# bigmat18/cuda-mesh-voxelization

Hardware: AMD Instinct MI355X
Metric: Mvoxels/s (voxelize+JFA) at N=512, bunny 1.35M tris (higher is better)
Workload: dtype f32

## Files before the change

cuda_mesh_voxelization_amd/build.py:

```python
from __future__ import annotations

import os
import shutil
import subprocess

PKG = os.path.dirname(os.path.abspath(__file__))
ROOT = os.path.dirname(PKG)
CSRC = os.path.join(PKG, "csrc")
LIB = os.path.join(PKG, "libvphip.so")
CLI = os.path.join(PKG, "vpcli")

HIP_SOURCES = ["capi.hip", "vox.hip", "csg.hip", "jfa_seed.hip", "jfa_first_two.hip", "jfa_dense.hip", "extract.hip", "multi.hip", "cvox.hip", "fill.hip", "morph.hip", "components.hip", "surfnets.hip", "edt.hip", "meshdist.hip", "isonets.hip", "winding.hip", "thickness.hip", "octree.hip", "skeleton.hip", "geodesic.hip"]
DENSE_PARTS = 10
HOOK_SOURCES = ["vox.hip", "multi.hip", "cvox.hip", "meshdist.hip"]
HOOKS_LIB = os.path.join(PKG, "libvphip_hooks.so")
HIP_FLAGS = ["--offload-arch=gfx950", "-O3", "-std=c++17", "-ffp-contract=off", "-fPIC", "-shared",
             "-Wall", "-Wno-unused-function"]


def _hipcc() -> str:
    exe = shutil.which("hipcc") or "/opt/rocm/bin/hipcc"
    if not os.path.exists(exe):
        raise RuntimeError("hipcc not found: cannot build libvphip.so")
    return exe


def _newer(target: str, sources) -> bool:
    if not os.path.exists(target):
        return True
    t = os.path.getmtime(target)
    return any(os.path.getmtime(s) > t for s in sources)


def _jobs(n: int) -> int:
    env = os.environ.get("VP_BUILD_JOBS")
    if env:
        return max(1, min(int(env), n))
    return max(1, min(8, max(2, (os.cpu_count() or 4) - 1), n))


def build_lib(force: bool = False, verbose: bool = False, hooks: bool = False) -> str:
    srcs = [os.path.join(CSRC, s) for s in HIP_SOURCES]
    deps = srcs + [os.path.join(CSRC, "vp_internal.h"), os.path.join(CSRC, "jfa_common.h"), os.path.join(CSRC, "wg_scan.h"), os.path.join(CSRC, "skeleton_simple.h"), os.path.join(ROOT, "include", "vphip.h")]
    objdir = os.path.join(PKG, "build")
    flags = [f for f in HIP_FLAGS if f != "-shared"]

    def link(objs, out):
        cmd = [_hipcc(), "--offload-arch=gfx950", "-shared", "-fPIC"] + objs + ["-o", out]
        if verbose:
            print(" ".join(cmd))
        subprocess.check_call(cmd)

    objs = []
    for s_ in srcs:
        base = os.path.basename(s_)
        if base == "jfa_dense.hip":
            objs += [os.path.join(objdir, "jfa_dense.hip.part%d.o" % part) for part in range(1, DENSE_PARTS + 1)]
        else:
            objs.append(os.path.join(objdir, base + ".o"))
    if force or _newer(LIB, deps) or (hooks and (force or _newer(HOOKS_LIB, deps + [LIB])) and not all(os.path.exists(o) for o in objs)):
        from concurrent.futures import ThreadPoolExecutor
        os.makedirs(objdir, exist_ok=True)
        cmds = []
        for s_ in srcs:
            base = os.path.basename(s_)
# ... 45 lines not shown
```

cuda_mesh_voxelization_amd/capi.py:

```python
from __future__ import annotations

import ctypes
import os

PKG = os.path.dirname(os.path.abspath(__file__))
LIB_PATH = os.environ.get("VPHIP_LIB") or os.path.join(PKG, "libvphip.so")
HOOKS_LIB_PATH = os.path.join(PKG, "libvphip_hooks.so")

ALGO_NAIVE, ALGO_TILED = 1, 2
OP_VOID, OP_UNION, OP_INTERSECTION, OP_DIFFERENCE = 0, 1, 2, 3
MORPH_DILATE, MORPH_ERODE, MORPH_OPEN, MORPH_CLOSE = 0, 1, 2, 3
EDT_SEEDS_SET, EDT_SEEDS_UNSET, EDT_SEEDS_BORDER = 0, 1, 2
EDT_NONE = 0xFFFFFFFF
MESH_NONE = 0xFFFFFFFF
ISO_LINEAR, ISO_SIGNED_SQUARE = 0, 1
CONN_6, CONN_26 = 6, 26
SKEL_KERNEL, SKEL_CURVE = 0, 1
GEO_6, GEO_26, GEO_CHAMFER = 0, 1, 2
GEO_NONE = 0xFFFFFFFF
COMP_KEEP_LARGEST, COMP_MIN_VOXELS = 0, 1
EXTRACT_SET, EXTRACT_EXPOSED, EXTRACT_FACES = 0, 1, 2
MULTI_HALO, MULTI_GHOST, MULTI_HYBRID, MULTI_TRANSPOSE = 0, 1, 2, 3

KERNELS = ["vox_setup", "vox_scan", "vox_scatter", "vox_tile", "vox_naive", "vox_fill",
# ... 388 lines not shown

    def release(self):
        check(lib().vp_ctx_release(self._h))

    def jfa_init(self, frame: Frame, d_words: int, d_below, d_above, d_ids: int):
        check(lib().vp_jfa_init(self._h, ctypes.byref(frame), _vp(d_words), _vp(d_below or None),
                                _vp(d_above or None), _vp(d_ids)))

    def jfa_pass(self, frame: Frame, k: int, d_in: int, d_minus, d_plus, d_out: int, algo: int = ALGO_TILED):
        check(lib().vp_jfa_pass(self._h, ctypes.byref(frame), k, _vp(d_in), _vp(d_minus or None),
                                _vp(d_plus or None), _vp(d_out), algo))

    def jfa_finalize(self, frame: Frame, d_words: int, d_ids: int, fill: float, d_sdf: int):
        check(lib().vp_jfa_finalize(self._h, ctypes.byref(frame), _vp(d_words), _vp(d_ids), fill, _vp(d_sdf)))

    def jfa_last_pass(self, frame: Frame, d_in: int, d_minus, d_plus, d_scratch: int, d_words: int, fill: float, d_sdf: int,
                      algo: int = ALGO_TILED):
        check(lib().vp_jfa_last_pass(self._h, ctypes.byref(frame), _vp(d_in), _vp(d_minus or None), _vp(d_plus or None),
                                     _vp(d_scratch), _vp(d_words), fill, _vp(d_sdf), algo))

    def jfa_can_start_from_mask(self, frame: Frame, algo: int = ALGO_TILED) -> bool:
        return bool(lib().vp_jfa_can_start_from_mask(ctypes.byref(frame), algo))

    def jfa_can_fuse_first_two(self, frame: Frame, algo: int = ALGO_TILED) -> bool:
        return bool(lib().vp_jfa_can_fuse_first_two(ctypes.byref(frame), algo))

    def jfa_window_bytes(self, frame: Frame, planes: int) -> int:
        return int(lib().vp_jfa_window_bytes(ctypes.byref(frame), planes))

    def jfa_window_span(self, frame: Frame, planes: int, p0: int, p1: int):
        off, nb = (_sz * 2)(), (_sz * 2)()
        check(lib().vp_jfa_window_span(ctypes.byref(frame), planes, p0, p1, off, nb))
        return [(int(off[i]), int(nb[i])) for i in range(2) if nb[i]]

    def jfa_window_clear(self, frame: Frame, win: Window):
        check(lib().vp_jfa_window_clear(self._h, ctypes.byref(frame), ctypes.byref(win)))

    def jfa_window_init(self, frame: Frame, d_words: int, d_below, d_above, win: Window):
        check(lib().vp_jfa_window_init(self._h, ctypes.byref(frame), _vp(d_words), _vp(d_below or None), _vp(d_above or None), ctypes.byref(win)))

    def jfa_window_first_pass(self, frame: Frame, d_border_grid: int, win: Window):
        check(lib().vp_jfa_window_first_pass(self._h, ctypes.byref(frame), _vp(d_border_grid), ctypes.byref(win)))

    def jfa_window_first_two(self, frame: Frame, d_border_grid: int, win: Window):
        check(lib().vp_jfa_window_first_two(self._h, ctypes.byref(frame), _vp(d_border_grid), ctypes.byref(win)))

    def jfa_window_pass(self, frame: Frame, k: int, win_in: Window, win_out: Window, stride=None):
        check(lib().vp_jfa_window_pass(self._h, ctypes.byref(frame), k, ctypes.byref(win_in), ctypes.byref(win_out), k if stride is None else stride))

    def jfa_window_last_pass(self, frame: Frame, win_in: Window, win_scratch: Window, d_words_region: int, fill: float, d_sdf_region: int, stride: int = 1):
        check(lib().vp_jfa_window_last_pass(self._h, ctypes.byref(frame), ctypes.byref(win_in), ctypes.byref(win_scratch), stride,
                                            _vp(d_words_region), fill, _vp(d_sdf_region)))

    @staticmethod
    def jfa_cyclic_passes(frame: Frame, ranks: int) -> int:
        return int(lib().vp_jfa_cyclic_passes(ctypes.byref(frame), ranks))

    def jfa_window_first_two_cyclic(self, frame: Frame, d_border_grid: int, win: Window, ranks: int, rank: int):
        check(lib().vp_jfa_window_first_two_cyclic(self._h, ctypes.byref(frame), _vp(d_border_grid), ctypes.byref(win), ranks, rank))

    def jfa_window_pass_cyclic(self, frame: Frame, k: int, win_in: Window, win_out: Window, ranks: int, rank: int):
        check(lib().vp_jfa_window_pass_cyclic(self._h, ctypes.byref(frame), k, ctypes.byref(win_in), ctypes.byref(win_out), ranks, rank))

    def jfa_window_interleave(self, frame: Frame, win_in: Window, win_out: Window, ranks: int, count: int):
        check(lib().vp_jfa_window_interleave(self._h, ctypes.byref(frame), ctypes.byref(win_in), ctypes.byref(win_out), ranks, count))

    def surface(self, frame: Frame, d_words: int, d_below, d_above, d_border: int):
        check(lib().vp_surface(self._h, ctypes.byref(frame), _vp(d_words), _vp(d_below or None),
                               _vp(d_above or None), _vp(d_border)))

    def extract_count(self, frame: Frame, d_words: int, mode: int) -> int:
        n = ctypes.c_uint64()
        check(lib().vp_extract_count(self._h, ctypes.byref(frame), _vp(d_words), mode, ctypes.byref(n)))
        return int(n.value)

    def extract(self, frame: Frame, d_words: int, mode: int, d_sdf, d_records: int, d_values, capacity: int):
        check(lib().vp_extract(self._h, ctypes.byref(frame), _vp(d_words), mode, _vp(d_sdf or None), _vp(d_records),
                               _vp(d_values or None), capacity))

    def surfnets_count(self, frame: Frame, d_words: int, algo: int = ALGO_TILED):
        nv, nq = ctypes.c_uint64(), ctypes.c_uint64()
        check(lib().vp_surfnets_count(self._h, ctypes.byref(frame), _vp(d_words), algo, ctypes.byref(nv), ctypes.byref(nq)))
        return int(nv.value), int(nq.value)

    def surfnets(self, frame: Frame, d_words: int, algo: int, iterations: int, d_cells: int, d_xyz: int, d_quads: int,
                 vertex_capacity: int, quad_capacity: int):
        check(lib().vp_surfnets(self._h, ctypes.byref(frame), _vp(d_words), algo, iterations, _vp(d_cells or None), _vp(d_xyz or None),
                                _vp(d_quads or None), vertex_capacity, quad_capacity))

    def isonets(self, frame: Frame, d_field: int, transform: int = ISO_SIGNED_SQUARE, iso: float = 0.0, iterations: int = 0,
                normals: bool = False, algo: int = ALGO_TILED):
        nv, nq = ctypes.c_uint64(), ctypes.c_uint64()
        check(lib().vp_isonets(self._h, ctypes.byref(frame), _vp(d_field or None), transform, iso, iterations, 1 if normals else 0, algo,
                               ctypes.byref(nv), ctypes.byref(nq)))
        return int(nv.value), int(nq.value)

    def isonets_result(self):
        c, x, m, q = _vp(), _vp(), _vp(), _vp()
        nv, nq = ctypes.c_uint64(), ctypes.c_uint64()
        check(lib().vp_isonets_result(self._h, ctypes.byref(c), ctypes.byref(x), ctypes.byref(m), ctypes.byref(q), ctypes.byref(nv),
                                      ctypes.byref(nq)))
        return c.value or 0, x.value or 0, m.value or 0, q.value or 0, int(nv.value), int(nq.value)

    def winding(self, frame: Frame, d_xyz: int, nverts: int, d_tri: int, ntris: int, beta: float = 2.0, level: float = 0.5,
                algo: int = ALGO_TILED, count: bool = False):
        c = ctypes.c_uint64()
# ... 285 lines not shown
```

cuda_mesh_voxelization_amd/csrc/capi.hip:

```cpp
#include "vp_internal.h"

#include <algorithm>
#include <cmath>
#include <cstdarg>
#include <cstdio>
#include <cstring>
#include <initializer_list>

namespace vp {

static thread_local char g_err[512] = "";

int set_error(int code, const char* fmt, ...)
{
    va_list ap;
    va_start(ap, fmt);
    vsnprintf(g_err, sizeof(g_err), fmt, ap);
    va_end(ap);
    return code;
}

int hip_fail(hipError_t e, const char* what, const char* file, int line)
{
    snprintf(g_err, sizeof(g_err), "[%s:%d] HIP Assert: %s (%s)", file, line, hipGetErrorString(e), what);
// ... 664 lines not shown
        VP_TRY(reserve(ctx, ctx->jfa_work, vp_jfa_workspace_bytes(f)));
        if (ctx->jfa_work.ptr != before) ctx->jfa_started.valid = false;
        d_work = ctx->jfa_work.ptr;
        work_bytes = ctx->jfa_work.bytes;
    } else if (work_bytes < vp_jfa_workspace_bytes(f)) {
        return set_error(VP_ERR_INVALID, "%s: workspace too small", who);
    }
    return 0;
}

static bool jfa_tile_sequence(const Frame& fr, int algo) { return jfa_can_fuse_first_two(fr, algo) && fr.n / 4 >= 1; }

int vp_jfa_start(vp_ctx* ctx, const vp_frame* f, const uint32_t* d_words, void* d_work, size_t work_bytes, int algo)
{
    const bool explicitWork = d_work != nullptr;
    VP_TRY(jfa_check(ctx, f, d_words, d_work, work_bytes, algo, "vp_jfa_start"));
    const Frame fr = make_frame(f);
    const size_t volBytes = vp_grid_voxels(f) * vp_jfa_id_bytes(f);
    char* a = (char*)d_work;
    const bool mask = jfa_tile_sequence(fr, algo);
    ctx->jfa_started.valid = false;
    if (explicitWork) grid_written(ctx, d_work, vp_jfa_workspace_bytes(f));
    if (mask) VP_TRY(launch_jfa_init(ctx, fr, d_words, nullptr, nullptr, nullptr, (uint32_t*)(a + 2 * volBytes)));
    else      VP_TRY(launch_jfa_init(ctx, fr, d_words, nullptr, nullptr, a, nullptr));
    ctx->jfa_started = {true, mask, f->n, algo, d_work, work_bytes, d_words};
    return 0;
}

int vp_jfa_run(vp_ctx* ctx, const vp_frame* f, const uint32_t* d_words, float fill_unset, float* d_sdf,
               void* d_work, size_t work_bytes, int algo)
{
    if (!d_sdf) return set_error(VP_ERR_INVALID, "vp_jfa_run: null argument");
    VP_TRY(check_aligned("vp_jfa_run", {d_sdf}));
    const bool explicitWork = d_work != nullptr;
    VP_TRY(jfa_check(ctx, f, d_words, d_work, work_bytes, algo, "vp_jfa_run"));
    VP_TRY(check_fill(fill_unset, "vp_jfa_run"));
    const Frame fr = make_frame(f);
    const size_t volBytes = vp_grid_voxels(f) * vp_jfa_id_bytes(f);
    char* a = (char*)d_work;
    char* b = a + volBytes;
    uint32_t k = f->n / 2;
    const bool wantMask = jfa_tile_sequence(fr, algo);
    const vp_ctx::JfaStarted st = ctx->jfa_started;
    ctx->jfa_started.valid = false;
    if (!st.valid || st.n != f->n || st.algo != algo || st.work != d_work || st.words != d_words || st.mask != wantMask)
        return set_error(VP_ERR_INVALID, "vp_jfa_run: call vp_jfa_start with the same grid, frame, algo and workspace first");
    if (explicitWork) grid_written(ctx, d_work, vp_jfa_workspace_bytes(f));
    grid_written(ctx, d_sdf, vp_grid_voxels(f) * 4);
    if (wantMask) {
        IdWin wa, wb;
        wa.base = a; wb.base = b; wa.planes = wb.planes = f->n; wa.at = wb.at = 0;
        VP_TRY(launch_win_first_two(ctx, fr, (const uint32_t*)(b + volBytes), wa));
        for (k /= 4; k >= 1; k /= 2) {
            if (k == 1) return launch_win_pass(ctx, fr, 1, wa, wb, 1, d_words, fill_unset, d_sdf);
            VP_TRY(launch_win_pass(ctx, fr, k, wa, wb, k, nullptr, 0.0f, nullptr));
            std::swap(wa, wb);
        }
        return set_error(VP_ERR_INVALID, "vp_jfa_run: internal: no last pass");
    }
    for (; k >= 1; k /= 2) {
        if (k == 1 && jfa_pass_can_fuse_final(fr, k, algo))
            return launch_jfa_pass_ex(ctx, fr, k, a, nullptr, nullptr, b, algo, d_words, fill_unset, d_sdf);
        VP_TRY(launch_jfa_pass(ctx, fr, k, a, nullptr, nullptr, b, algo));
        char* t = a; a = b; b = t;
    }
    return launch_jfa_final(ctx, fr, d_words, a, fill_unset, d_sdf);
}

int vp_jfa(vp_ctx* ctx, const vp_frame* f, const uint32_t* d_words, float fill_unset, float* d_sdf,
           void* d_work, size_t work_bytes, int algo)
{
    if (!d_sdf) return set_error(VP_ERR_INVALID, "vp_jfa: null argument");
    VP_TRY(check_aligned("vp_jfa", {d_sdf}));
    VP_TRY(check_fill(fill_unset, "vp_jfa"));
    VP_TRY(vp_jfa_start(ctx, f, d_words, d_work, work_bytes, algo));
    return vp_jfa_run(ctx, f, d_words, fill_unset, d_sdf, d_work, work_bytes, algo);
}

size_t vp_jfa_state_bytes(const vp_frame* f, int algo)
{
    if (!f || check_frame(f, "vp_jfa_state_bytes", false) != 0) return 0;
    return (algo == VP_ALGO_TILED && win_compact(f->n)) ? 5 : vp_jfa_id_bytes(f);
}

int vp_jfa_last_shapes(const vp_ctx* ctx, vp_jfa_shape* out, int cap)
{
    if (!ctx) return 0;
    for (int i = 0; out && i < ctx->dense_shape_count && i < cap; ++i) out[i] = ctx->dense_shapes[i];
    return ctx->dense_shape_count;
}

int vp_jfa_can_start_from_mask(const vp_frame* f, int algo)
{
    return (f && check_frame(f, "vp_jfa_can_start_from_mask", false) == 0 && jfa_can_start_from_mask(make_frame(f), algo)) ? 1 : 0;
}

int vp_jfa_can_fuse_first_two(const vp_frame* f, int algo)
{
    return (f && check_frame(f, "vp_jfa_can_fuse_first_two", false) == 0 && jfa_can_fuse_first_two(make_frame(f), algo)) ? 1 : 0;
}

int vp_jfa_last_pass(vp_ctx* ctx, const vp_frame* f, const void* d_in, const void* d_minus, const void* d_plus,
                     void* d_scratch, const uint32_t* d_words, float fill_unset, float* d_sdf, int algo)
{
    if (ctx) ctx->dense_shape_count = 0;
    if (!ctx || !d_in || !d_scratch || !d_words || !d_sdf || d_in == d_scratch)
        return set_error(VP_ERR_INVALID, "vp_jfa_last_pass: bad buffers");
// ... 157 lines not shown
        return set_error(VP_ERR_INVALID, "%s: %llu planes at index %u do not fit a window of %u planes", who, (unsigned long long)planes, out->at, out->planes);
    if (overlaps(in->d_ids, win_bytes(f->n, in->planes), out->d_ids, win_bytes(f->n, out->planes))) return set_error(VP_ERR_INVALID, "%s: the two windows overlap", who);
    IdWin wi, wo;
    wi.base = (char*)in->d_ids; wi.planes = in->planes; wi.at = 0;
    wo.base = (char*)out->d_ids; wo.planes = out->planes; wo.at = out->at;
    window_written(ctx, out);
    return launch_win_interleave(ctx, f->n, wi, wo, ranks, count);
}

static void pass_reach(const vp_frame* f, uint32_t k, uint32_t stride, uint32_t& below, uint32_t& above)
{
    if (stride == k) {
        below = std::min(k, f->z0);
        above = std::min(k, f->n - f->z1);
    } else {
        below = f->z1 > k ? stride : 0;
        above = f->z0 + k < f->n ? stride : 0;
    }
}

static int window_pass(vp_ctx* ctx, const vp_frame* f, uint32_t k, const vp_window* in, const vp_window* out, uint32_t stride,
                       const uint32_t* d_words, float fill, float* d_sdf, const char* who)
{
    if (ctx) ctx->dense_shape_count = 0;
    if (!in || !out || !in->d_ids || !out->d_ids || in->d_ids == out->d_ids) return set_error(VP_ERR_INVALID, "%s: bad windows", who);
    if (in->planes != out->planes || in->at != out->at) return set_error(VP_ERR_INVALID, "%s: the two windows must have the same planes / at", who);
    if (f && f->n && overlaps(in->d_ids, win_bytes(f->n, in->planes), out->d_ids, win_bytes(f->n, out->planes)))
        return set_error(VP_ERR_INVALID, "%s: the two windows overlap", who);
    if (!f || k == 0 || k >= f->n) return set_error(VP_ERR_INVALID, "%s: step %u out of range", who, k);
    if (stride == 0 || (stride != k && (k < f->z1 - f->z0 || stride < f->z1 - f->z0)))
        return set_error(VP_ERR_INVALID, "%s: stride %u: either the step itself or, for a step of at least the slab height, the distance of the slabs in the window", who, stride);
    uint32_t below = 0, above = 0;
    pass_reach(f, k, stride, below, above);
    IdWin wi, wo;
    VP_TRY(window_check(ctx, f, in, who, below, above, wi));
    VP_TRY(window_check(ctx, f, out, who, 0, 0, wo));
    window_written(ctx, out);
    if (d_sdf) grid_written(ctx, d_sdf, vp_grid_voxels(f) * 4);
    return launch_win_pass(ctx, make_frame(f), k, wi, wo, stride, d_words, fill, d_sdf);
}

int vp_jfa_window_pass(vp_ctx* ctx, const vp_frame* f, uint32_t k, const vp_window* in, const vp_window* out, uint32_t stride)
{
    return window_pass(ctx, f, k, in, out, stride, nullptr, 0.0f, nullptr, "vp_jfa_window_pass");
}

int vp_jfa_window_last_pass(vp_ctx* ctx, const vp_frame* f, const vp_window* in, const vp_window* scratch, uint32_t stride,
                            const uint32_t* d_words_region, float fill_unset, float* d_sdf_region)
{
    if (!d_words_region || !d_sdf_region) return set_error(VP_ERR_INVALID, "vp_jfa_window_last_pass: null argument");
    VP_TRY(check_aligned("vp_jfa_window_last_pass", {d_words_region, d_sdf_region}));
    VP_TRY(check_fill(fill_unset, "vp_jfa_window_last_pass"));
    return window_pass(ctx, f, 1, in, scratch, stride, d_words_region, fill_unset, d_sdf_region, "vp_jfa_window_last_pass");
}

int vp_extract_count(vp_ctx* ctx, const vp_frame* f, const uint32_t* d_words, int mode, uint64_t* h_count)
{
    if (!ctx || !d_words) return set_error(VP_ERR_INVALID, "vp_extract_count: null argument");
    VP_TRY(bind_device(ctx));
    VP_TRY(check_frame(f, "vp_extract_count", true));
    if (mode < VP_EXTRACT_SET || mode > VP_EXTRACT_FACES) return set_error(VP_ERR_INVALID, "vp_extract_count: mode %d", mode);
    return launch_extract_count(ctx, make_frame(f), d_words, mode, h_count);
}

int vp_extract(vp_ctx* ctx, const vp_frame* f, const uint32_t* d_words, int mode, const float* d_sdf,
               uint64_t* d_records, float* d_values, size_t capacity)
{
    if (!ctx || !d_words || (!d_records && capacity)) return set_error(VP_ERR_INVALID, "vp_extract: null argument");
    if ((d_values != nullptr) != (d_sdf != nullptr)) return set_error(VP_ERR_INVALID, "vp_extract: d_sdf and d_values go together");
    VP_TRY(bind_device(ctx));
    VP_TRY(check_frame(f, "vp_extract", true));
    if (mode < VP_EXTRACT_SET || mode > VP_EXTRACT_FACES) return set_error(VP_ERR_INVALID, "vp_extract: mode %d", mode);
    const size_t cnt = (size_t)std::min<uint64_t>(capacity, ctx->ext_total);
    if (cnt) {
        grid_written(ctx, d_records, cnt * 8);
        grid_written(ctx, d_values, cnt * 4);
    }
    return launch_extract_write(ctx, make_frame(f), d_words, mode, d_sdf, d_records, d_values, capacity);
}

static int check_surfnets(const vp_frame* f, const char* who)
{
    VP_TRY(check_frame(f, who, false));
    VP_TRY(check_whole(f, who));
    if (f->n > 1024) return set_error(VP_ERR_UNSUPPORTED, "%s: n=%u is not served (32 <= n <= 1024: cell indices are 32-bit)", who, f->n);
    return 0;
}

int vp_surfnets_count(vp_ctx* ctx, const vp_frame* f, const uint32_t* d_words, int algo, uint64_t* h_vertices, uint64_t* h_quads)
{
    const char* who = "vp_surfnets_count";
    if (!ctx || !d_words || !h_vertices || !h_quads) return set_error(VP_ERR_INVALID, "%s: null argument", who);
    VP_TRY(bind_device(ctx));
    VP_TRY(check_surfnets(f, who));
    VP_TRY(check_algo(who, algo));
    VP_TRY(check_aligned(who, {d_words}));
    return launch_surfnets_count(ctx, f->n, d_words, algo, h_vertices, h_quads);
}

int vp_surfnets(vp_ctx* ctx, const vp_frame* f, const uint32_t* d_words, int algo, uint32_t iterations, uint64_t* d_cells, float* d_xyz,
                uint32_t* d_quads, size_t vertex_capacity, size_t quad_capacity)
{
    const char* who = "vp_surfnets";
    if (!ctx || !d_words) return set_error(VP_ERR_INVALID, "%s: null argument", who);
    VP_TRY(bind_device(ctx));
    VP_TRY(check_surfnets(f, who));
// ... 623 lines not shown
```

cuda_mesh_voxelization_amd/csrc/jfa_common.h:

```cpp
#pragma once
#include "vp_internal.h"
#include <algorithm>
#include <cstdlib>
#include <type_traits>

#pragma clang fp contract(off)

namespace vp {
namespace {

__device__ __forceinline__ uint32_t scr(uint32_t i) { return i ^ ((i >> 5) & 31u); }

__device__ __forceinline__ void udivmod(uint32_t a, uint32_t b, uint32_t& q, uint32_t& r)
{
    if ((b & (b - 1u)) == 0u) { q = a >> (uint32_t)__builtin_ctz(b); r = a & (b - 1u); }
    else { q = a / b; r = a % b; }
}

struct FastDiv {
    uint32_t d, m, s1, s2;
    __device__ __forceinline__ void divmod(uint32_t a, uint32_t& q, uint32_t& r) const
    {
        const uint32_t t = __umulhi(m, a);
        q = (t + ((a - t) >> s1)) >> s2;
// ... 53 lines not shown
    static constexpr int kTabZ = 3072;
    static constexpr uint32_t kMask = 0x1FFCu;
    static constexpr uint32_t kNoneWord = 0xFFFFF800u;
    static constexpr uint32_t kNoneBit = 4u;
    static constexpr uint32_t kNoneByte = 4u;
    __device__ static __forceinline__ T none() { return make_uint2(kNoneWord, kNoneByte); }
    __device__ static __forceinline__ bool is_none(T a) { return (a.y & kNoneBit) != 0u; }
    __device__ static __forceinline__ T pack(uint32_t x, uint32_t y, uint32_t z)
    {
        const uint32_t sz = scr(z);
        return make_uint2(x | (scr(y) << 11) | ((sz & 1023u) << 22), (sz >> 10) << 1);
    }
    __device__ static __forceinline__ T from64(uint2 a)
    {
        if (a.x == 0xFFFFFFFFu) return none();
        const uint32_t sz = (a.x >> 2) & 2047u, sy = (a.y >> 2) & 2047u;
        return make_uint2((a.x >> 13) | (sy << 11) | ((sz & 1023u) << 22), (sz >> 10) << 1);
    }
    __device__ static __forceinline__ uint32_t xoff(T a) { return (a.x & 0x7FFu) << 2; }
    __device__ static __forceinline__ uint32_t zoff(T a) { return ((a.x >> 20) & 0xFFCu) | (a.y << 11); }
    __device__ static __forceinline__ uint32_t yoff(T a) { return (a.x >> 9) & kMask; }
    __device__ static __forceinline__ uint32_t zt2(T a) { return a.y & 2u; }
};

__device__ __forceinline__ float axis_pos(float o, uint32_t i, float vs) { return o + ((float)(int)i * vs); }

template <class ID>
__device__ __forceinline__ float seed_distance(const Frame& f, typename ID::T id, float px, float py, float pz)
{
    const float sx = axis_pos(f.ox, ID::xoff(id) >> 2, f.vs);
    const float sy = axis_pos(f.oy, scr(ID::yoff(id) >> 2), f.vs);
    const float sz = axis_pos(f.oz, scr(ID::zoff(id) >> 2), f.vs);
    return ((sx - px) * (sx - px)) + ((sy - py) * (sy - py)) + ((sz - pz) * (sz - pz));
}

__device__ __forceinline__ __amdgpu_buffer_rsrc_t row_resource(const void* row, uint32_t bytes)
{
    return __builtin_amdgcn_make_buffer_rsrc(const_cast<void*>(row), 0, (int)bytes, 0x00020000);
}
__device__ __forceinline__ void row_load(uint32_t& o, __amdgpu_buffer_rsrc_t r, uint32_t byte_off)
{
    o = __builtin_amdgcn_raw_buffer_load_b32(r, (int)byte_off, 0, 0);
}
__device__ __forceinline__ void row_load(uint2& o, __amdgpu_buffer_rsrc_t r, uint32_t byte_off)
{
    const auto v = __builtin_amdgcn_raw_buffer_load_b64(r, (int)byte_off, 0, 0);
    o = make_uint2(v[0], v[1]);
}
__device__ __forceinline__ uint32_t row_load_u8(__amdgpu_buffer_rsrc_t r, uint32_t byte_off)
{
    return (uint32_t)__builtin_amdgcn_raw_buffer_load_b8(r, (int)byte_off, 0, 0);
}
__device__ __forceinline__ float lds_f32(const char* p) { return *reinterpret_cast<const float*>(p); }
template <int AUX = 0>
__device__ __forceinline__ void row_store(uint32_t v, __amdgpu_buffer_rsrc_t r, uint32_t byte_off)
{
    __builtin_amdgcn_raw_buffer_store_b32(v, r, (int)byte_off, 0, AUX);
}
template <int AUX = 0>
__device__ __forceinline__ void row_store(float v, __amdgpu_buffer_rsrc_t r, uint32_t byte_off)
{
    __builtin_amdgcn_raw_buffer_store_b32(__float_as_uint(v), r, (int)byte_off, 0, AUX);
}
template <int AUX = 0>
__device__ __forceinline__ void row_store(uint2 v, __amdgpu_buffer_rsrc_t r, uint32_t byte_off)
{
    typedef uint32_t u32x2 __attribute__((ext_vector_type(2)));
    const u32x2 t = {v.x, v.y};
    __builtin_amdgcn_raw_buffer_store_b64(t, r, (int)byte_off, 0, AUX);
}
template <int AUX = 0>
__device__ __forceinline__ void row_store_u8(uint32_t v, __amdgpu_buffer_rsrc_t r, uint32_t byte_off)
{
    __builtin_amdgcn_raw_buffer_store_b8((unsigned char)v, r, (int)byte_off, 0, AUX);
}
__device__ __forceinline__ const char* opaque_uniform(const char* p)
{
    uint64_t v = reinterpret_cast<uint64_t>(p);
    asm volatile("" : "+s"(v));
    return reinterpret_cast<const char*>(v);
}
__device__ __forceinline__ size_t opaque_uniform(size_t v)
{
    asm volatile("" : "+s"(v));
    return v;
}
__device__ __forceinline__ void pin(float& a) { asm volatile("" : "+v"(a)); }
__device__ __forceinline__ void pin(uint32_t& a) { asm volatile("" : "+v"(a)); }
__device__ __forceinline__ void pin(uint2& a) { asm volatile("" : "+v"(a.x), "+v"(a.y)); }

typedef uint32_t u32x2 __attribute__((ext_vector_type(2)));

__device__ __forceinline__ double min_f64(double a, double b)
{
    double r;
    asm("v_min_f64 %0, %1, %2" : "=v"(r) : "v"(a), "v"(b));
    return r;
}
__device__ __forceinline__ float min3_f32(float a, float b, float c)
{
    float r;
    asm("v_min3_f32 %0, %1, %2, %3" : "=v"(r) : "v"(a), "v"(b), "v"(c));
    return r;
}

__device__ __forceinline__ float min_f32(float a, float b)
// ... 21 lines not shown
```

cuda_mesh_voxelization_amd/csrc/jfa_dense.hip:

```cpp
#include "jfa_common.h"

namespace vp {
namespace {

template <class ID> constexpr bool final_mask_global() { return ID::kTab > 512; }
constexpr int kStoreAux = 2;
template <int PM>
__device__ __forceinline__ float from_partner(float v)
{
    constexpr int ctrl = PM == 1 ? 0xB1 : PM == 2 ? 0x4E : PM == 4 ? 0x141 : 0x128;
    return __builtin_bit_cast(float, __builtin_amdgcn_update_dpp(0, __builtin_bit_cast(int, v), ctrl, 0xf, 0xf, true));
}
template <class ID, int RY, int NT, bool FINAL>
constexpr int dense_waves()
{
    return std::is_same<ID, IdC>::value ? 4 : RY > 4 ? 4 : (FINAL && !final_mask_global<ID>()) ? (ID::kTab == 512 ? 5 : 4) : (ID::kTab == 512 || NT == 512) ? 6 : 4;
}
template <class ID, int RY, int CH, int NT, bool FINAL, int PM, int CLOSED = 0, bool FULL = false, bool CYC = false>
__global__ void __launch_bounds__(NT, (dense_waves<ID, RY, NT, FINAL>()))
jfa_pass_dense(Frame f, uint32_t kArg, uint32_t ka, const char* __restrict__ in, const char* __restrict__ inB, char* __restrict__ out, char* __restrict__ outB,
               const char* __restrict__ none_row, const uint32_t* __restrict__ words, float fill, float* __restrict__ sdf,
               uint32_t tilesY, uint32_t tiles, uint32_t splitTiles, uint32_t cyc)
{
    static_assert(!CYC || !FINAL, "the last pass (k = 1) is never a multiple of the rank count");
    using T = typename ID::T;
    constexpr bool CPT = std::is_same<ID, IdC>::value;
    constexpr uint32_t IDB = 4u;
    constexpr int TAB = ID::kTab;
    constexpr int PXT = CPT ? TAB : TAB + 1;
    constexpr int TABZ = CPT ? IdC::kTabZ : TAB;
    constexpr int HY = (CLOSED & 1) ? 0 : 1;
    constexpr bool CZ = (CLOSED & 2) != 0;
    constexpr int NR = RY + 2 * HY;
    static_assert(!CLOSED || !FINAL, "closed tiles: id passes");
    constexpr int NC = PM ? 2 : 3;
    constexpr int NI = NR * NC;
    constexpr int CHT = CPT ? 1 : CH;
    using B = typename std::conditional<FINAL, float, double>::type;
    __shared__ float PX[PXT];
    __shared__ float TY[RY][TAB];
    __shared__ float TZ[CHT][TABZ];
    __shared__ uint32_t RB[CPT ? (CH + 2) * NR : 1];
    constexpr bool GM = final_mask_global<ID>();
    __shared__ uint32_t WM[(FINAL && !GM) ? RY * CH * (TAB / 32) : 1];

    const int N = (int)f.n;
    const uint32_t k = FINAL ? 1u : kArg;
    const int K = (int)k;
    const int zsh = CYC ? (int)(cyc & 31u) : 0, zoff = CYC ? (int)(cyc >> 8) : 0;
    const int KZ = CYC ? K >> zsh : K, NZ = CYC ? N >> zsh : N;
    auto zglobal = [&](int l) { return CYC ? zoff + (l << zsh) : l; };
    const int nzl = (int)(f.z1 - f.z0);
    const uint32_t tid = threadIdx.x;
    const int nresY = min(K, N);
    const bool rev = ((31 - __builtin_clz(k)) & 1) != 0;
    uint32_t lin = blockIdx.x;
    const uint32_t total = tiles;
    uint32_t xpart = 0, xparts = 1;
    if (lin >= total - splitTiles) {
// ... 568 lines not shown
```

cuda_mesh_voxelization_amd/csrc/vp_internal.h:

```cpp
#pragma once

#include <hip/hip_runtime.h>
#include <cstddef>
#include <cstdint>
#include <vector>

#include "../../include/vphip.h"

namespace vp {

constexpr uint32_t kNone9 = 0xFF9FF200u;
constexpr uint32_t kNone10 = 0xFFDFFC00u;
constexpr int kTile = 8;
constexpr int kRecDwords = 20;

struct Frame {
    uint32_t n;
    uint32_t w;
    uint32_t z0, z1;
    float vs, ox, oy, oz;
};

inline Frame make_frame(const vp_frame* f)
{
// ... 147 lines not shown
int launch_morph(vp_ctx* ctx, uint32_t n, const uint32_t* d_words, uint32_t* d_out, int op, uint32_t radius, int algo);
int launch_edt(vp_ctx* ctx, const Frame& f, const uint32_t* d_words, int seeds, uint32_t* d_dist, int algo);
int launch_edt_sdf(vp_ctx* ctx, const Frame& f, const uint32_t* d_words, float fill, float* d_sdf, int algo);
int launch_edt_morph(vp_ctx* ctx, const Frame& f, const uint32_t* d_words, uint32_t* d_out, int op, uint32_t radius, int algo);
int launch_edt_thresh(vp_ctx* ctx, uint32_t n, const uint32_t* d_dist, uint32_t* d_out, uint32_t r2, int greater);
int launch_thickness(vp_ctx* ctx, const Frame& f, const uint32_t* d_words, uint32_t rmax, uint32_t thin2, int algo, uint64_t* h_thin_count);
int launch_octree(vp_ctx* ctx, const Frame& f, const uint32_t* d_words, int algo, uint64_t* h_nodes);
int launch_octree_expand(vp_ctx* ctx, const Frame& f, const uint32_t* d_nodes, uint64_t nodes, uint32_t* d_words, int algo);
int octree_validate(const uint32_t* h_nodes, uint64_t nodes, uint32_t n);
int launch_skeleton(vp_ctx* ctx, const Frame& f, const uint32_t* d_words, const uint32_t* d_anchor, int mode, uint32_t max_iters, int algo,
                    uint64_t* h_stats);
int launch_skeleton_table(vp_ctx* ctx, int algo, uint32_t* d_table);
void skeleton_table_cpu(int algo, uint32_t* h_table);
int launch_geodesic(vp_ctx* ctx, const Frame& f, const uint32_t* d_mask, const uint32_t* d_seeds, int metric, int algo, uint64_t* h_stats);
int launch_mesh_distance(vp_ctx* ctx, const Frame& f, const float* d_xyz, size_t nverts, const uint32_t* d_tri, size_t ntris,
                         const uint32_t* d_sign, uint32_t band, float* d_dist, uint32_t* d_nearest, int algo);
int launch_winding(vp_ctx* ctx, const Frame& f, const float* d_xyz, size_t nverts, const uint32_t* d_tri, size_t ntris, float beta, float level,
                   int algo, uint64_t* h_inside_count);
int launch_components_label(vp_ctx* ctx, uint32_t n, const uint32_t* d_words, uint32_t* d_labels, int conn, int algo, uint32_t* h_count);
int launch_components_sizes(vp_ctx* ctx, uint32_t n, const uint32_t* d_labels, uint32_t count, uint32_t* d_sizes);
int launch_components_filter(vp_ctx* ctx, uint32_t n, const uint32_t* d_words, uint32_t* d_out, int conn, int mode, uint32_t param, int algo,
                             uint32_t* h_count, uint64_t* h_kept);
int launch_surfnets_count(vp_ctx* ctx, uint32_t n, const uint32_t* d_words, int algo, uint64_t* h_vertices, uint64_t* h_quads);
struct IsoField { const float* d_field; int transform; float iso; float* d_normals; };
int launch_surfnets_write(vp_ctx* ctx, uint32_t n, const uint32_t* d_words, int algo, uint32_t iterations, uint64_t* d_cells, float* d_xyz,
                          uint32_t* d_quads, const IsoField* iso = nullptr);
int launch_isonets(vp_ctx* ctx, uint32_t n, const float* d_field, int transform, float iso, uint32_t iterations, bool want_normals, int algo);
int launch_iso_place(vp_ctx* ctx, uint32_t n, int algo, const IsoField& iso, const uint64_t* d_cells, const uint32_t* index, float* d_xyz,
                     size_t nverts);
int launch_csg(vp_ctx* ctx, uint32_t* d_a, const uint32_t* d_b, size_t nwords, int op);
int launch_stream_copy(vp_ctx* ctx, void* d_dst, const void* d_src, size_t bytes);
size_t jfa_id_bytes(const Frame& f);
int launch_jfa_init(vp_ctx* ctx, const Frame& f, const uint32_t* d_words, const uint32_t* below,
                    const uint32_t* above, void* d_ids, uint32_t* d_border_words);
int launch_jfa_pass(vp_ctx* ctx, const Frame& f, uint32_t k, const void* d_in, const void* d_minus,
                    const void* d_plus, void* d_out, int algo);
bool jfa_pass_can_fuse_final(const Frame& f, uint32_t k, int algo);
int launch_jfa_pass_ex(vp_ctx* ctx, const Frame& f, uint32_t k, const void* d_in, const void* d_minus,
                       const void* d_plus, void* d_out, int algo, const uint32_t* d_words, float fill, float* d_sdf);
int launch_jfa_final(vp_ctx* ctx, const Frame& f, const uint32_t* d_words, const void* d_ids,
                     float fill, float* d_sdf);
bool jfa_can_start_from_mask(const Frame& f, int algo);
bool jfa_can_fuse_first_two(const Frame& f, int algo);
int launch_win_init(vp_ctx* ctx, const Frame& f, const uint32_t* d_words, const uint32_t* below, const uint32_t* above, const IdWin& out);
int launch_win_first_pass(vp_ctx* ctx, const Frame& f, const uint32_t* d_border, const IdWin& out);
int launch_win_clear(vp_ctx* ctx, uint32_t n, const IdWin& w);
int launch_win_pass(vp_ctx* ctx, const Frame& f, uint32_t k, const IdWin& in, const IdWin& out, uint32_t stride,
                    const uint32_t* d_words, float fill, float* d_sdf);
#define VP_DENSE_DECL(NAME) int NAME(vp_ctx* ctx, const Frame& f, uint32_t k, const IdWin& in, const IdWin& out, uint32_t stride, const uint32_t* d_words, float fill, float* d_sdf)
VP_DENSE_DECL(launch_dense_id9_pass);  VP_DENSE_DECL(launch_dense_id9_last);
VP_DENSE_DECL(launch_dense_id10_pass); VP_DENSE_DECL(launch_dense_id10_last);
VP_DENSE_DECL(launch_dense_idc_pass);  VP_DENSE_DECL(launch_dense_idc_last);
#undef VP_DENSE_DECL
int launch_win_first_two(vp_ctx* ctx, const Frame& f, const uint32_t* d_border, const IdWin& out, uint32_t ranks = 1, uint32_t rank = 0);
uint32_t jfa_cyclic_passes(uint32_t n, uint32_t ranks);
int launch_win_pass_cyclic(vp_ctx* ctx, const Frame& f, uint32_t k, const IdWin& in, const IdWin& out, uint32_t ranks, uint32_t rank);
#define VP_CYCLIC_DECL(NAME) int NAME(vp_ctx* ctx, const Frame& f, uint32_t k, const IdWin& in, const IdWin& out, uint32_t ranks, uint32_t rank)
VP_CYCLIC_DECL(launch_cyclic_id9_pass); VP_CYCLIC_DECL(launch_cyclic_id10_pass); VP_CYCLIC_DECL(launch_cyclic_idc_pass);
#undef VP_CYCLIC_DECL
int launch_win_interleave(vp_ctx* ctx, uint32_t n, const IdWin& in, const IdWin& out, uint32_t ranks, uint32_t count);
int launch_extract_count(vp_ctx* ctx, const Frame& f, const uint32_t* d_words, int mode, uint64_t* h_count);
int launch_extract_write(vp_ctx* ctx, const Frame& f, const uint32_t* d_words, int mode, const float* d_sdf,
                         uint64_t* d_records, float* d_values, size_t capacity);

}
```

Measured before the change: 51160.

## Add dedicated lane-vectorized kernel for the final JFA pass on whole grids

Adds a specialized kernel for the final k=1 JFA pass on whole power-of-two grids (256/512/1024). Each thread owns four consecutive x voxels loaded with 16-byte buffer loads and writes signed distances with 16-byte stores. The kernel rolls through z planes, reusing neighbour rows across planes, and precomputes squared y/z distance tables in LDS. It replaces the generic dense final pass whenever the id window and sdf are 16-byte aligned, trading higher register pressure and more code for fewer memory transactions and less redundant arithmetic.

```diff
diff --git a/cuda_mesh_voxelization_amd/build.py b/cuda_mesh_voxelization_amd/build.py
--- a/cuda_mesh_voxelization_amd/build.py
+++ b/cuda_mesh_voxelization_amd/build.py
@@ -10,7 +10,7 @@
 LIB = os.path.join(PKG, "libvphip.so")
 CLI = os.path.join(PKG, "vpcli")
 
-HIP_SOURCES = ["capi.hip", "vox.hip", "csg.hip", "jfa_seed.hip", "jfa_first_two.hip", "jfa_dense.hip", "extract.hip", "multi.hip", "cvox.hip", "fill.hip", "morph.hip", "components.hip", "surfnets.hip", "edt.hip", "meshdist.hip", "isonets.hip", "winding.hip", "thickness.hip", "octree.hip", "skeleton.hip", "geodesic.hip"]
+HIP_SOURCES = ["capi.hip", "vox.hip", "csg.hip", "jfa_seed.hip", "jfa_first_two.hip", "jfa_dense.hip", "jfa_last.hip", "extract.hip", "multi.hip", "cvox.hip", "fill.hip", "morph.hip", "components.hip", "surfnets.hip", "edt.hip", "meshdist.hip", "isonets.hip", "winding.hip", "thickness.hip", "octree.hip", "skeleton.hip", "geodesic.hip"]
 DENSE_PARTS = 10
 HOOK_SOURCES = ["vox.hip", "multi.hip", "cvox.hip", "meshdist.hip"]
 HOOKS_LIB = os.path.join(PKG, "libvphip_hooks.so")
diff --git a/cuda_mesh_voxelization_amd/capi.py b/cuda_mesh_voxelization_amd/capi.py
--- a/cuda_mesh_voxelization_amd/capi.py
+++ b/cuda_mesh_voxelization_amd/capi.py
@@ -464,6 +464,11 @@
         check(lib().vp_jfa_window_last_pass(self._h, ctypes.byref(frame), ctypes.byref(win_in), ctypes.byref(win_scratch), stride,
                                             _vp(d_words_region), fill, _vp(d_sdf_region)))
 
+    def jfa_last_pass_lanes(self, frame: Frame, win_in: Window, d_words: int, fill: float, d_sdf: int):
+        fn = lib().vp_jfa_last_pass_lanes
+        fn.restype, fn.argtypes = ctypes.c_int, [_vp, ctypes.POINTER(Frame), ctypes.POINTER(Window), _vp, ctypes.c_float, _vp]
+        check(fn(self._h, ctypes.byref(frame), ctypes.byref(win_in), _vp(d_words), fill, _vp(d_sdf)))
+
     @staticmethod
     def jfa_cyclic_passes(frame: Frame, ranks: int) -> int:
         return int(lib().vp_jfa_cyclic_passes(ctypes.byref(frame), ranks))
diff --git a/cuda_mesh_voxelization_amd/csrc/capi.hip b/cuda_mesh_voxelization_amd/csrc/capi.hip
--- a/cuda_mesh_voxelization_amd/csrc/capi.hip
+++ b/cuda_mesh_voxelization_amd/csrc/capi.hip
@@ -740,7 +740,10 @@
         wa.base = a; wb.base = b; wa.planes = wb.planes = f->n; wa.at = wb.at = 0;
         VP_TRY(launch_win_first_two(ctx, fr, (const uint32_t*)(b + volBytes), wa));
         for (k /= 4; k >= 1; k /= 2) {
-            if (k == 1) return launch_win_pass(ctx, fr, 1, wa, wb, 1, d_words, fill_unset, d_sdf);
+            if (k == 1) {
+                if (jfa_last_lanes_serves(fr, wa, d_sdf)) return launch_jfa_last_lanes(ctx, fr, wa, d_words, fill_unset, d_sdf);
+                return launch_win_pass(ctx, fr, 1, wa, wb, 1, d_words, fill_unset, d_sdf);
+            }
             VP_TRY(launch_win_pass(ctx, fr, k, wa, wb, k, nullptr, 0.0f, nullptr));
             std::swap(wa, wb);
         }
@@ -1004,6 +1007,25 @@
     VP_TRY(check_aligned("vp_jfa_window_last_pass", {d_words_region, d_sdf_region}));
     VP_TRY(check_fill(fill_unset, "vp_jfa_window_last_pass"));
     return window_pass(ctx, f, 1, in, scratch, stride, d_words_region, fill_unset, d_sdf_region, "vp_jfa_window_last_pass");
+}
+
+int vp_jfa_last_pass_lanes(vp_ctx* ctx, const vp_frame* f, const vp_window* in, const uint32_t* d_words, float fill_unset, float* d_sdf)
+{
+    const char* who = "vp_jfa_last_pass_lanes";
+    if (ctx) ctx->dense_shape_count = 0;
+    if (!ctx || !d_words || !d_sdf) return set_error(VP_ERR_INVALID, "%s: null argument", who);
+    VP_TRY(bind_device(ctx));
+    VP_TRY(check_frame(f, who, false));
+    VP_TRY(check_fill(fill_unset, who));
+    const uint32_t n = f->n;
+    if ((n != 256 && n != 512 && n != 1024) || f->z0 != 0 || f->z1 != n)
+        return set_error(VP_ERR_UNSUPPORTED, "%s: whole grids of 256, 512 or 1024 voxels per side only", who);
+    IdWin wi;
+    VP_TRY(window_check(ctx, f, in, who, 0, 0, wi));
+    const Frame fr = make_frame(f);
+    if (!jfa_last_lanes_serves(fr, wi, d_sdf)) return set_error(VP_ERR_UNSUPPORTED, "%s: the id window and the sdf must be 16-byte aligned", who);
+    grid_written(ctx, d_sdf, vp_grid_voxels(f) * 4);
+    return launch_jfa_last_lanes(ctx, fr, wi, d_words, fill_unset, d_sdf);
 }
 
 int vp_extract_count(vp_ctx* ctx, const vp_frame* f, const uint32_t* d_words, int mode, uint64_t* h_count)
diff --git a/cuda_mesh_voxelization_amd/csrc/jfa_common.h b/cuda_mesh_voxelization_amd/csrc/jfa_common.h
--- a/cuda_mesh_voxelization_amd/csrc/jfa_common.h
+++ b/cuda_mesh_voxelization_amd/csrc/jfa_common.h
@@ -129,6 +129,7 @@
     return (uint32_t)__builtin_amdgcn_raw_buffer_load_b8(r, (int)byte_off, 0, 0);
 }
 __device__ __forceinline__ float lds_f32(const char* p) { return *reinterpret_cast<const float*>(p); }
+constexpr int kStoreAux = 2;
 template <int AUX = 0>
 __device__ __forceinline__ void row_store(uint32_t v, __amdgpu_buffer_rsrc_t r, uint32_t byte_off)
 {
diff --git a/cuda_mesh_voxelization_amd/csrc/jfa_dense.hip b/cuda_mesh_voxelization_amd/csrc/jfa_dense.hip
--- a/cuda_mesh_voxelization_amd/csrc/jfa_dense.hip
+++ b/cuda_mesh_voxelization_amd/csrc/jfa_dense.hip
@@ -4,7 +4,6 @@
 namespace {
 
 template <class ID> constexpr bool final_mask_global() { return ID::kTab > 512; }
-constexpr int kStoreAux = 2;
 template <int PM>
 __device__ __forceinline__ float from_partner(float v)
 {
diff --git a/cuda_mesh_voxelization_amd/csrc/jfa_last.hip b/cuda_mesh_voxelization_amd/csrc/jfa_last.hip
--- /dev/null
+++ b/cuda_mesh_voxelization_amd/csrc/jfa_last.hip
@@ -0,0 +1,243 @@
+#include "jfa_common.h"
+
+namespace vp {
+namespace {
+
+constexpr int kLanesNT = 512;
+
+template <int I, int E, class F>
+__device__ __forceinline__ void static_for(F&& fn)
+{
+    if constexpr (I <= E) { fn(std::integral_constant<int, I>{}); static_for<I + 1, E>(fn); }
+}
+
+template <class ID, int N, int V, int RY, int CH>
+__global__ void __launch_bounds__(kLanesNT, 4)
+jfa_last_lanes(Frame f, const char* __restrict__ in, const char* __restrict__ none_row, const uint32_t* __restrict__ words, float fill,
+               float* __restrict__ sdf)
+{
+    constexpr int NT = kLanesNT;
+    constexpr int TAB = ID::kTab;
+    constexpr int LR = N / V;
+    constexpr int G = NT / LR;
+    constexpr int TR = G * RY;
+    constexpr int NR = RY + 2, NC = V + 2, NI = NR * NC;
+    constexpr uint32_t W = N / 32;
+    constexpr uint32_t rowBytes = (uint32_t)N * 4u;
+    constexpr size_t planeBytes = (size_t)N * rowBytes;
+    constexpr uint32_t tilesY = N / TR, tiles = tilesY * (N / CH);
+    static_assert(V == 4, "16-byte loads and stores");
+    static_assert(LR % 64 == 0 && NT % LR == 0 && G >= 1, "a row is a whole number of waves, a workgroup a whole number of rows");
+    static_assert(N % TR == 0 && N % CH == 0 && N <= TAB && tiles % 8 == 0, "whole tiles");
+    __shared__ float PX[TAB + 1];
+    __shared__ float TY[TR][TAB];
+    __shared__ float TZ[CH][TAB];
+
+    const uint32_t tid = threadIdx.x;
+    const uint32_t lin = (blockIdx.x & 7u) * (tiles >> 3) + (blockIdx.x >> 3);
+    const int ybase0 = (int)(lin % tilesY) * TR, zbase = (int)(lin / tilesY) * CH;
+    {
+        float py[TR], pz[CH];
+#pragma unroll
+        for (int j = 0; j < TR; ++j) py[j] = axis_pos(f.oy, ybase0 + j, f.vs);
+#pragma unroll
+        for (int j = 0; j < CH; ++j) pz[j] = axis_pos(f.oz, zbase + j, f.vs);
+        for (uint32_t i = tid; i < (uint32_t)(TAB + 1); i += NT) PX[i] = i < (uint32_t)N ? axis_pos(f.ox, i, f.vs) : INFINITY;
+        for (uint32_t i = tid; i < (uint32_t)TAB; i += NT) {
+            if (i < (uint32_t)N) {
+                const uint32_t si = scr(i);
+                const float sy = axis_pos(f.oy, i, f.vs), sz = axis_pos(f.oz, i, f.vs);
+#pragma unroll
+                for (int j = 0; j < TR; ++j) { const float d = sy - py[j]; TY[j][si] = d * d; }
+#pragma unroll
+                for (int j = 0; j < CH; ++j) { const float d = sz - pz[j]; TZ[j][si] = d * d; }
+            } else {
+#pragma unroll
+                for (int j = 0; j < TR; ++j) TY[j][i] = 0.0f;
+#pragma unroll
+                for (int j = 0; j < CH; ++j) TZ[j][i] = 0.0f;
+            }
+        }
+    }
+    __syncthreads();
+
+    const int g = __builtin_amdgcn_readfirstlane((int)(tid / LR));
+    const uint32_t x0 = (tid % LR) * V;
+    const int ybase = ybase0 + g * RY;
+    const char* tx = reinterpret_cast<const char*>(PX);
+    const char* ty = reinterpret_cast<const char*>(TY) + g * (RY * TAB * 4);
+    const char* tz = reinterpret_cast<const char*>(TZ);
+
+    float px[V];
+#pragma unroll
+    for (int v = 0; v < V; ++v) px[v] = PX[x0 + v];
+    const uint32_t xo = x0 * 4u;
+    const uint32_t xmo = x0 > 0u ? xo - 4u : xo;
+    const uint32_t xpo = x0 + V < (uint32_t)N ? xo + V * 4u : xo + (V - 1) * 4u;
+    const uint32_t mo = (x0 >> 5) << 2, mb = x0 & 31u;
+    uint32_t ro[NR];
+    bool yv[NR];
+#pragma unroll
+    for (int rr = 0; rr < NR; ++rr) {
+        const int ny = ybase + rr - 1;
+        yv[rr] = ny >= 0 && ny < N;
+        ro[rr] = (uint32_t)(yv[rr] ? ny : 0) * rowBytes;
+    }
+
+    struct Plane { const char* base; bool ok; };
+    auto plane_of = [&](int P) __attribute__((always_inline)) {
+        Plane pl;
+        const int zg = zbase + P;
+        pl.ok = zg >= 0 && zg < N;
+        pl.base = opaque_uniform(in + (size_t)(pl.ok ? zg : 0) * planeBytes);
+        return pl;
+    };
+    auto load_row = [&](const Plane& pl, int rr, uint32_t (&w)[NI]) __attribute__((always_inline)) {
+        const __amdgpu_buffer_rsrc_t b = row_resource((pl.ok && yv[rr]) ? pl.base + ro[rr] : none_row, rowBytes);
+        row_load(w[rr * NC], b, xmo);
+        const auto own = __builtin_amdgcn_raw_buffer_load_b128(b, (int)xo, 0, 0);
+#pragma unroll
+        for (int v = 0; v < V; ++v) w[rr * NC + 1 + v] = own[v];
+        row_load(w[rr * NC + NC - 1], b, xpo);
+    };
+
+    float best[RY][CH][V];
+    struct Dec { float sx; float dy2[RY]; float dz2[CH]; };
+    auto lookup = [&](int P, int rr, uint32_t id, Dec& d) __attribute__((always_inline)) {
+        const int alo = max(rr - 2, 0), ahi = min(rr, RY - 1), olo = max(P - 1, 0), ohi = min(P + 1, CH - 1);
+        d.sx = lds_f32(tx + ID::xoff(id));
+        const uint32_t yo = ID::yoff(id), zo = ID::zoff(id);
+#pragma unroll
+        for (int a = alo; a <= ahi; ++a) d.dy2[a] = lds_f32(ty + a * (TAB * 4) + yo);
+#pragma unroll
+        for (int o = olo; o <= ohi; ++o) d.dz2[o] = lds_f32(tz + o * (TAB * 4) + zo);
+    };
+    float hold[3][3];
+    auto steps = [&](int P, int rr, int c, const Dec& d) __attribute__((always_inline)) {
+        const int alo = max(rr - 2, 0), ahi = min(rr, RY - 1), olo = max(P - 1, 0), ohi = min(P + 1, CH - 1);
+        auto column = [&](int v, int role) __attribute__((always_inline)) {
+            const float dxv = d.sx - px[v];
+            const float dx2 = dxv * dxv;
+#pragma unroll
+            for (int a = alo; a <= ahi; ++a) {
+                const float pre = d.dy2[a] + dx2;
+#pragma unroll
+                for (int o = olo; o <= ohi; ++o) {
+                    const float dd = d.dz2[o] + pre;
+                    if (role == 0) hold[a - alo][o - olo] = dd;
+                    else if (role == 1) best[a][o][v] = min3_f32(best[a][o][v], hold[a - alo][o - olo], dd);
+                    else best[a][o][v] = min_f32(best[a][o][v], dd);
+                }
+            }
+        };
+        if (c >= 1 && c - 1 < V) column(c - 1, 1);
+        if (c < V) column(c, 0);
+        if (c >= 2) column(c - 2, 2);
+    };
+    auto scatter = [&](int P, uint32_t (&w)[NI]) __attribute__((always_inline)) {
+        const int olo = max(P - 1, 0), ohi = min(P + 1, CH - 1);
+        Plane next{nullptr, false};
+        const bool roll = P + 1 <= CH;
+        if (roll) next = plane_of(P + 1);
+        Dec d[2];
+        lookup(P, 0, w[0], d[0]);
+        static_for<0, NI - 1>([&](auto jc) __attribute__((always_inline)) {
+            constexpr int j = decltype(jc)::value, rr = j / NC, c = j % NC;
+            if constexpr (j + 1 < NI) lookup(P, (j + 1) / NC, w[j + 1], d[(j + 1) % 2]);
+            __builtin_amdgcn_sched_barrier(0);
+            steps(P, rr, c, d[j % 2]);
+            if (c == NC - 1) {
+                const int alo = max(rr - 2, 0), ahi = min(rr, RY - 1);
+#pragma unroll
+                for (int a = alo; a <= ahi; ++a)
+#pragma unroll
+                    for (int o = olo; o <= ohi; ++o)
+#pragma unroll
+                        for (int v = 0; v < V; ++v) pin(best[a][o][v]);
+                if (roll) load_row(next, rr, w);
+            }
+            __builtin_amdgcn_sched_barrier(0);
+        });
+    };
+
+    uint32_t w[NI];
+    {
+        const Plane first = plane_of(-1);
+#pragma unroll
+        for (int rr = 0; rr < NR; ++rr) load_row(first, rr, w);
+    }
+    static_for<-1, CH>([&](auto pc) __attribute__((always_inline)) {
+        constexpr int P = decltype(pc)::value;
+        if constexpr (P + 1 < CH) {
+#pragma unroll
+            for (int a = 0; a < RY; ++a)
+#pragma unroll
+                for (int v = 0; v < V; ++v) best[a][P + 1][v] = INFINITY;
+        }
+        uint32_t mw[RY] = {};
+        if constexpr (P >= 1) {
+            const char* wpl = opaque_uniform(reinterpret_cast<const char*>(words) + ((size_t)(zbase + P - 1) * N + ybase) * (size_t)(W * 4u));
+            const __amdgpu_buffer_rsrc_t wr = row_resource(wpl, (uint32_t)RY * W * 4u);
+#pragma unroll
+            for (int a = 0; a < RY; ++a) mw[a] = (uint32_t)__builtin_amdgcn_raw_buffer_load_b32(wr, (int)mo, (int)((uint32_t)a * W * 4u), 0);
+        }
+        scatter(P, w);
+        if constexpr (P >= 1) {
+            const char* spl = opaque_uniform(reinterpret_cast<const char*>(sdf) + ((size_t)(zbase + P - 1) * N + ybase) * (size_t)rowBytes);
+            const __amdgpu_buffer_rsrc_t sr = row_resource(spl, (uint32_t)RY * rowBytes);
+#pragma unroll
+            for (int a = 0; a < RY; ++a) {
+                const uint32_t bits = mw[a] >> mb;
+                uint32_t o[V];
+#pragma unroll
+                for (int v = 0; v < V; ++v) {
+                    const float b = best[a][P - 1][v];
+                    o[v] = __float_as_uint(((bits >> v) & 1u) ? b : copysignf(b, fill));
+                }
+                typedef uint32_t u32x4 __attribute__((ext_vector_type(4)));
+                const u32x4 t = {o[0], o[1], o[2], o[3]};
+                __builtin_amdgcn_raw_buffer_store_b128(t, sr, (int)(xo + (uint32_t)a * rowBytes), 0, kStoreAux);
+            }
+        }
+#pragma unroll
+        for (int a = 0; a < RY; ++a)
+#pragma unroll
+            for (int o = P; o <= P + 1; ++o)
+                if (o >= 0 && o < CH) {
+#pragma unroll
+                    for (int v = 0; v < V; ++v) pin(best[a][o][v]);
+                }
+    });
+}
+
+template <class ID, int N, int V, int RY, int CH>
+void launch_lanes(vp_ctx* ctx, const Frame& f, const char* in, const char* none_row, const uint32_t* d_words, float fill, float* d_sdf)
+{
+    constexpr uint32_t tiles = (uint32_t)(N / (kLanesNT / (N / V) * RY)) * (uint32_t)(N / CH);
+    hipLaunchKernelGGL((jfa_last_lanes<ID, N, V, RY, CH>), dim3(tiles), dim3(kLanesNT), 0, ctx->stream, f, in, none_row, d_words, fill, d_sdf);
+}
+
+}
+
+bool jfa_last_lanes_serves(const Frame& f, const IdWin& in, const float* d_sdf)
+{
+    const uint32_t n = f.n;
+    return (n == 256 || n == 512 || n == 1024) && f.z0 == 0 && f.z1 == n &&
+           ((reinterpret_cast<uintptr_t>(win_words(in, n, in.at)) | reinterpret_cast<uintptr_t>(d_sdf)) & 15u) == 0;
+}
+
+int launch_jfa_last_lanes(vp_ctx* ctx, const Frame& f, const IdWin& in, const uint32_t* d_words, float fill, float* d_sdf)
+{
+    ProfScope p(ctx, VP_K_JFA_LAST);
+    ctx->dense_shape_count = 0;
+    if (!jfa_last_lanes_serves(f, in, d_sdf)) return set_error(VP_ERR_UNSUPPORTED, "jfa_last_lanes: whole power-of-two grids of 256 .. 1024 voxels per side");
+    VP_TRY(ensure_none_rows(ctx));
+    const char* src = win_words(in, f.n, in.at);
+    if (f.n == 256)      launch_lanes<Id9, 256, 4, 2, 8>(ctx, f, src, (const char*)none_row_id9(ctx), d_words, fill, d_sdf);
+    else if (f.n == 512) launch_lanes<Id9, 512, 4, 4, 16>(ctx, f, src, (const char*)none_row_id9(ctx), d_words, fill, d_sdf);
+    else                 launch_lanes<Id10, 1024, 4, 4, 8>(ctx, f, src, (const char*)none_row_id10(ctx), d_words, fill, d_sdf);
+    VP_HIP(hipGetLastError());
+    return 0;
+}
+
+}
diff --git a/cuda_mesh_voxelization_amd/csrc/vp_internal.h b/cuda_mesh_voxelization_amd/csrc/vp_internal.h
--- a/cuda_mesh_voxelization_amd/csrc/vp_internal.h
+++ b/cuda_mesh_voxelization_amd/csrc/vp_internal.h
@@ -223,6 +223,8 @@
 VP_DENSE_DECL(launch_dense_id10_pass); VP_DENSE_DECL(launch_dense_id10_last);
 VP_DENSE_DECL(launch_dense_idc_pass);  VP_DENSE_DECL(launch_dense_idc_last);
 #undef VP_DENSE_DECL
+bool jfa_last_lanes_serves(const Frame& f, const IdWin& in, const float* d_sdf);
+int launch_jfa_last_lanes(vp_ctx* ctx, const Frame& f, const IdWin& in, const uint32_t* d_words, float fill, float* d_sdf);
 int launch_win_first_two(vp_ctx* ctx, const Frame& f, const uint32_t* d_border, const IdWin& out, uint32_t ranks = 1, uint32_t rank = 0);
 uint32_t jfa_cyclic_passes(uint32_t n, uint32_t ranks);
 int launch_win_pass_cyclic(vp_ctx* ctx, const Frame& f, uint32_t k, const IdWin& in, const IdWin& out, uint32_t ranks, uint32_t rank);
```

After: 51580, median of 6. Within noise of the previous version (+0.8%).
